# burchim/AVEC

Hardware: AMD Instinct MI355X
Metric: AV utterances/sec fwd+bwd (audio T=400, video 100x88x88) (higher is better)
Workload: dtype bf16

## Files before the change

avec_amd/csrc/wgrad_pairs.hip:

```cpp
#include "common.h"
#include "vec.h"
#include "avec_hip.h"

#ifndef WP_ABL
#define WP_ABL 0
#endif
typedef __attribute__((ext_vector_type(16))) float wp_f32x16;
typedef __attribute__((ext_vector_type(8))) __bf16 wp_bf16x8;
typedef short wp_v4s __attribute__((ext_vector_type(4)));

__device__ __attribute__((aligned(64))) unsigned char wp_zero16[64];

__device__ __forceinline__ void wp_glds16(const void* gsrc, unsigned lds_dst_uniform) {
  unsigned keep;
  asm volatile("s_mov_b32 %0, m0\n\ts_mov_b32 m0, %2\n\ts_nop 0\n\tglobal_load_lds_dwordx4 %1, off\n\ts_mov_b32 m0, %0" : "=&s"(keep) : "v"(gsrc), "s"(lds_dst_uniform) : "memory");
}
__device__ __forceinline__ uint2 wp_tr(const char* p) {
  typedef __attribute__((address_space(3))) wp_v4s* lp_t;
  return __builtin_bit_cast(uint2, __builtin_amdgcn_ds_read_tr16_b64_v4i16((lp_t)p));
}
struct WpFrag { uint2 lo, hi; };
__device__ __forceinline__ wp_f32x16 wp_mma(const WpFrag& a, const WpFrag& b, wp_f32x16 c) {
  chunk16 fa, fb; fa.w[0] = a.lo.x; fa.w[1] = a.lo.y; fa.w[2] = a.hi.x; fa.w[3] = a.hi.y; fb.w[0] = b.lo.x; fb.w[1] = b.lo.y; fb.w[2] = b.hi.x; fb.w[3] = b.hi.y;
  if (WP_ABL & 2) { asm volatile("" :: "v"(fa.w[0]), "v"(fa.w[1]), "v"(fa.w[2]), "v"(fa.w[3]), "v"(fb.w[0]), "v"(fb.w[1]), "v"(fb.w[2]), "v"(fb.w[3])); return c; }
  return __builtin_amdgcn_mfma_f32_32x32x16_bf16(__builtin_bit_cast(wp_bf16x8, fa), __builtin_bit_cast(wp_bf16x8, fb), c, 0, 0, 0);
}

struct WpArgs { const bf16* x; const bf16* dy; float* dw; int N, C, H, W; };

template <int H_, int W_, int KS_> struct WpGeom {
  static constexpr int H = H_, W = W_, KS = KS_;
  static constexpr int RWD = W | 1;
  static constexpr int RWX = W;
  static constexpr int ROWS = 16 * KS;
  static constexpr int DYB = ROWS * RWD * 128, XB = (ROWS + 2) * RWX * 256;
  static constexpr int DYI = (DYB + 1023) / 1024, XI = (XB + 1023) / 1024;
  static constexpr int DPL = (DYI + 7) / 8, XPL = (XI + 7) / 8;
  static constexpr int STAGE = (DYI + XI) * 1024;
  static constexpr int PAIRS = 3 * (3 * W - 2);
};

__device__ __forceinline__ void wp_glds16_s(unsigned voff, const void* sbase, unsigned lds_dst_uniform) {
  unsigned keep;
  asm volatile("s_mov_b32 %0, m0\n\ts_mov_b32 m0, %3\n\ts_nop 0\n\tglobal_load_lds_dwordx4 %1, %2\n\ts_mov_b32 m0, %0" : "=&s"(keep) : "v"(voff), "s"(sbase), "s"(lds_dst_uniform) : "memory");
}
template <int OFF> __device__ __forceinline__ uint2 wp_tr_o(unsigned addr) {
  static_assert(OFF >= 0 && OFF < 65536, "ds offset field");
  uint2 v; asm volatile("ds_read_b64_tr_b16 %0, %1 offset:%2" : "=v"(v) : "v"(addr), "n"(OFF) : "memory"); return v;
}

struct WpRegs { WpFrag A[4]; WpFrag B[3]; };

template <typename G, int I> struct WpIt {
  static constexpr int W = G::W, s = I / W, xp = I % W, g = s * W + xp;
  static constexpr int N0 = 2 + 2 * ((xp == 0 ? 1 : 0) + (xp + 1 < W ? 1 : 0));
  static __device__ __forceinline__ void issue0(WpRegs& R, const unsigned (&aA)[2], const unsigned (&aB)[3][2]) {
    if constexpr (xp == 0) { R.A[g & 3].lo = wp_tr_o<(16 * s * G::RWD) * 128>(aA[0]); R.A[g & 3].hi = wp_tr_o<(16 * s * G::RWD) * 128>(aA[1]); }
    if constexpr (xp + 1 < W) { R.A[(g + 1) & 3].lo = wp_tr_o<(16 * s * G::RWD + xp + 1) * 128>(aA[0]); R.A[(g + 1) & 3].hi = wp_tr_o<(16 * s * G::RWD + xp + 1) * 128>(aA[1]); }
    R.B[0].lo = wp_tr_o<(16 * s * G::RWX + xp) * 256>(aB[0][0]); R.B[0].hi = wp_tr_o<(16 * s * G::RWX + xp) * 256>(aB[0][1]);
  }
  template <int KH> static __device__ __forceinline__ void issueB(WpRegs& R, const unsigned (&aB)[3][2]) {
    R.B[KH].lo = wp_tr_o<(16 * s * G::RWX + xp) * 256>(aB[KH][0]); R.B[KH].hi = wp_tr_o<(16 * s * G::RWX + xp) * 256>(aB[KH][1]);
  }
  static __device__ __forceinline__ void arrived0(WpRegs& R) {
    if constexpr (xp == 0) asm volatile("" : "+v"(R.A[g & 3].lo), "+v"(R.A[g & 3].hi));
    if constexpr (xp + 1 < W) asm volatile("" : "+v"(R.A[(g + 1) & 3].lo), "+v"(R.A[(g + 1) & 3].hi));
    asm volatile("" : "+v"(R.B[0].lo), "+v"(R.B[0].hi));
  }
};

template <typename G, int I>
__device__ __forceinline__ void wp_iter(WpRegs& R, wp_f32x16 (&acc)[9], unsigned (&m0)[4], unsigned (&m2)[4], const int oyb, const bool hi_half, const unsigned (&aA)[2], const unsigned (&aB)[3][2]) {
  typedef WpIt<G, I> It;
  constexpr int H = G::H, W = G::W, NIT = G::KS * W, g = It::g;
  constexpr bool more = I + 1 < NIT;
  constexpr int N0N = more ? WpIt<G, more ? I + 1 : I>::N0 : 0;
  if constexpr (It::xp == 0) {
    constexpr unsigned PAT = 1u | (1u << H) | (2 * H < 16 ? 1u << ((2 * H) & 15) : 0u) | (3 * H < 16 ? 1u << ((3 * H) & 15) : 0u) | (4 * H < 16 ? 1u << ((4 * H) & 15) : 0u);
    unsigned ml0[2][4], ml2[2][4];
#pragma unroll
    for (int hh = 0; hh < 2; ++hh) {
      int bs = oyb + (8 * hh + 16 * It::s) % H; bs = bs >= H ? bs - H : bs;
      const int e0 = bs == 0 ? 0 : H - bs, e2 = e0 == 0 ? H - 1 : e0 - 1;
      const unsigned b0 = (WP_ABL & 8) ? 0u : (PAT << e0), b2 = (WP_ABL & 8) ? 0u : (PAT << e2);
#pragma unroll
      for (int dd = 0; dd < 4; ++dd) {
        ml0[hh][dd] = ~((((b0 >> (2 * dd)) & 1u) * 0xffffu) | (((b0 >> (2 * dd + 1)) & 1u) * 0xffff0000u));
        ml2[hh][dd] = ~((((b2 >> (2 * dd)) & 1u) * 0xffffu) | (((b2 >> (2 * dd + 1)) & 1u) * 0xffff0000u));
      }
    }
#pragma unroll
    for (int dd = 0; dd < 4; ++dd) { m0[dd] = hi_half ? ml0[1][dd] : ml0[0][dd]; m2[dd] = hi_half ? ml2[1][dd] : ml2[0][dd]; }
  }
  asm volatile("s_waitcnt lgkmcnt(4)" ::: "memory");
  It::arrived0(R);
  R.B[0].lo.x &= m0[0]; R.B[0].lo.y &= m0[1]; R.B[0].hi.x &= m0[2]; R.B[0].hi.y &= m0[3];
  if constexpr (It::xp + 1 < W) acc[0] = wp_mma(R.A[(g + 1) & 3], R.B[0], acc[0]);
  acc[1] = wp_mma(R.A[g & 3], R.B[0], acc[1]);
  if constexpr (It::xp >= 1) acc[2] = wp_mma(R.A[(g - 1) & 3], R.B[0], acc[2]);
  __builtin_amdgcn_sched_barrier(0);
  if constexpr (more) WpIt<G, more ? I + 1 : I>::issue0(R, aA, aB);
  asm volatile("s_waitcnt lgkmcnt(%0)" ::"n"(2 + N0N) : "memory");
  asm volatile("" : "+v"(R.B[1].lo), "+v"(R.B[1].hi));
  if constexpr (It::xp + 1 < W) acc[3] = wp_mma(R.A[(g + 1) & 3], R.B[1], acc[3]);
  acc[4] = wp_mma(R.A[g & 3], R.B[1], acc[4]);
  if constexpr (It::xp >= 1) acc[5] = wp_mma(R.A[(g - 1) & 3], R.B[1], acc[5]);
  __builtin_amdgcn_sched_barrier(0);
  if constexpr (more) WpIt<G, more ? I + 1 : I>::template issueB<1>(R, aB);
  asm volatile("s_waitcnt lgkmcnt(%0)" ::"n"(more ? N0N + 2 : 0) : "memory");
  asm volatile("" : "+v"(R.B[2].lo), "+v"(R.B[2].hi));
  R.B[2].lo.x &= m2[0]; R.B[2].lo.y &= m2[1]; R.B[2].hi.x &= m2[2]; R.B[2].hi.y &= m2[3];
  if constexpr (It::xp + 1 < W) acc[6] = wp_mma(R.A[(g + 1) & 3], R.B[2], acc[6]);
  acc[7] = wp_mma(R.A[g & 3], R.B[2], acc[7]);
  if constexpr (It::xp >= 1) acc[8] = wp_mma(R.A[(g - 1) & 3], R.B[2], acc[8]);
  __builtin_amdgcn_sched_barrier(0);
  if constexpr (more) { WpIt<G, more ? I + 1 : I>::template issueB<2>(R, aB); wp_iter<G, more ? I + 1 : I>(R, acc, m0, m2, oyb, hi_half, aA, aB); }
}

template <typename G>
__device__ __attribute__((noinline)) void wp_body(const WpArgs a_, char* const smem_, const int kind_, const int s_begin_, const int s_end_) {
  constexpr int H = G::H, W = G::W, RWD = G::RWD, RWX = G::RWX, ROWS = G::ROWS;
  auto uni = [](const void* p) { const unsigned long long v = (unsigned long long)p;
    return (const void*)(((unsigned long long)(unsigned)__builtin_amdgcn_readfirstlane((int)(v >> 32)) << 32) | (unsigned)__builtin_amdgcn_readfirstlane((int)(unsigned)v)); };
  WpArgs a; a.x = (const bf16*)uni(a_.x); a.dy = (const bf16*)uni(a_.dy); a.dw = (float*)uni(a_.dw);
  a.N = __builtin_amdgcn_readfirstlane(a_.N); a.C = __builtin_amdgcn_readfirstlane(a_.C); a.H = a_.H; a.W = a_.W;
  char* const smem = (char*)uni(smem_);
  const int kind = __builtin_amdgcn_readfirstlane(kind_), s_begin = __builtin_amdgcn_readfirstlane(s_begin_), s_end = __builtin_amdgcn_readfirstlane(s_end_);
  const int tid = threadIdx.x, lane = tid & 63, wave = __builtin_amdgcn_readfirstlane(tid >> 6);
  const int C = a.C;
  const int nci = C >> 7, cog = kind / nci, cig = kind - cog * nci;
  typedef __attribute__((address_space(3))) void* lptr_t;
  const unsigned lds0 = (unsigned)(uintptr_t)(lptr_t)smem;
  const int NR = a.N * H;

  unsigned dpl[G::DPL], xpl[G::XPL];
  auto dslot = [&](const int k, int& rr, bool& used) {
    const int S = (wave + 8 * k) * 64 + lane, pix = S >> 3, cpos = S & 7;
    rr = pix / RWD; const int xx = pix - rr * RWD, c = cpos ^ (4 * ((rr >> 1) & 1));
    used = rr < ROWS && xx < W;
    return (unsigned)(((rr * W + xx) * C + cog * 64 + c * 8) * 2);
  };
  auto xslot = [&](const int k, int& rr, bool& used) {
    const int S = (wave + 8 * k) * 64 + lane, pix = S >> 4, cpos = S & 15;
    rr = pix / RWX; const int xx = pix - rr * RWX, c = cpos ^ (4 * (rr & 3));
    used = rr < ROWS + 2;
    return (unsigned)(((rr * W + xx) * C + cig * 128 + c * 8) * 2);
  };
#pragma unroll
  for (int k = 0; k < G::DPL; ++k) { int rr; bool u; const unsigned o = dslot(k, rr, u); dpl[k] = u ? o : 0u; }
#pragma unroll
  for (int k = 0; k < G::XPL; ++k) { int rr; bool u; const unsigned o = xslot(k, rr, u); xpl[k] = u ? o : 0u; }
  auto load_stage = [&](const int q, const int par) {
    const int rs = q * ROWS;
    const unsigned d0 = lds0 + par * G::STAGE, x0 = d0 + G::DYI * 1024;
    const char* dyb = (const char*)(a.dy + (long long)rs * W * C); const char* xb = (const char*)(a.x + (long long)(rs - 1) * W * C);
    if (rs >= 1 && rs + ROWS + 1 <= NR) {
#pragma unroll
      for (int k = 0; k < G::DPL; ++k) { if (wave + 8 * k >= G::DYI) break; wp_glds16_s(dpl[k], dyb, d0 + (wave + 8 * k) * 1024); }
#pragma unroll
      for (int k = 0; k < G::XPL; ++k) { if (wave + 8 * k >= G::XI) break; wp_glds16_s(xpl[k], xb, x0 + (wave + 8 * k) * 1024); }
    } else {
#pragma unroll
      for (int k = 0; k < G::DPL; ++k) {
        if (wave + 8 * k >= G::DYI) break;
        int rr; bool u; const unsigned o = dslot(k, rr, u);
        wp_glds16((u && rs + rr < NR) ? (const void*)(dyb + o) : (const void*)wp_zero16, d0 + (wave + 8 * k) * 1024);
      }
#pragma unroll
      for (int k = 0; k < G::XPL; ++k) {
        if (wave + 8 * k >= G::XI) break;
        int rr; bool u; const unsigned o = xslot(k, rr, u); const int r = rs - 1 + rr;
        wp_glds16((u && r >= 0 && r < NR) ? (const void*)(xb + o) : (const void*)wp_zero16, x0 + (wave + 8 * k) * 1024);
      }
    }
  };

  const int cot = wave & 1, ciq = wave >> 1;
  const int g4 = lane >> 4, t = lane & 15;
  unsigned aA[2], aB[3][2];
#pragma unroll
  for (int h = 0; h < 2; ++h) {
    const int krow = 8 * (g4 >> 1) + 4 * h + (t >> 2);
    aA[h] = lds0 + krow * RWD * 128 + (((2 * cot + (g4 & 1)) ^ (2 * ((krow >> 1) & 1))) << 5) + (t & 3) * 8;
#pragma unroll
    for (int kh = 0; kh < 3; ++kh) {
      const int rr = krow + kh;
      aB[kh][h] = lds0 + G::DYI * 1024 + rr * RWX * 256 + (((2 * ciq + (g4 & 1)) ^ (2 * (rr & 3))) << 5) + (t & 3) * 8;
    }
  }
  wp_f32x16 acc[9];
#pragma unroll
  for (int j = 0; j < 9; ++j)
#pragma unroll
    for (int r = 0; r < 16; ++r) acc[j][r] = 0.f;

  int q = s_begin;
  int par = 0;
  load_stage(q, 0);
  for (; q < s_end; ++q, par ^= 1) {
    asm volatile("s_waitcnt vmcnt(0)" ::: "memory");
    __builtin_amdgcn_s_barrier();
    asm volatile("" ::: "memory");
    WpRegs R; unsigned m0[4], m2[4];
    WpIt<G, 0>::issue0(R, aA, aB); WpIt<G, 0>::template issueB<1>(R, aB); WpIt<G, 0>::template issueB<2>(R, aB);
    if (q + 1 < s_end && !(WP_ABL & 1)) load_stage(q + 1, par ^ 1);
    const int oyb = (int)(((unsigned)q * (unsigned)ROWS) % (unsigned)H);
    wp_iter<G, 0>(R, acc, m0, m2, oyb, lane >= 32, aA, aB);
    const unsigned dlt = par ? (unsigned)-G::STAGE : (unsigned)G::STAGE;
#pragma unroll
    for (int h = 0; h < 2; ++h) { aA[h] += dlt; aB[0][h] += dlt; aB[1][h] += dlt; aB[2][h] += dlt; }
  }
#pragma unroll
  for (int j = 0; j < 9; ++j)
#pragma unroll
    for (int r = 0; r < 16; ++r) {
      const int co = cog * 64 + cot * 32 + (r & 3) + 8 * (r >> 2) + 4 * (lane >> 5), ci = cig * 128 + ciq * 32 + (lane & 31);
      if (WP_ABL & 4) { if (acc[j][r] == 1234.5f) a.dw[(long long)co * 9 * C + j * C + ci] = acc[j][r]; } else
      atomicAdd(a.dw + (long long)co * 9 * C + j * C + ci, acc[j][r]);
    }
  __builtin_amdgcn_s_barrier();
}

typedef WpGeom<11, 11, 1> WpG11;
typedef WpGeom<6, 6, 2> WpG6;
typedef WpGeom<3, 3, 4> WpG3;
static constexpr size_t wp_max3(size_t a, size_t b, size_t c) { return a > b ? (a > c ? a : c) : (b > c ? b : c); }
static constexpr size_t WP_LDS = wp_max3(2 * WpG11::STAGE, 2 * WpG6::STAGE, 2 * WpG3::STAGE);
static_assert(WP_LDS <= 160 * 1024, "two stages must fit the LDS");

struct WpGroup { WpArgs it[AVEC_WGRAD_GROUP_MAX]; long long cum[AVEC_WGRAD_GROUP_MAX + 1]; int stages[AVEC_WGRAD_GROUP_MAX], wt[AVEC_WGRAD_GROUP_MAX], ranges[AVEC_WGRAD_GROUP_MAX]; int n; };
__global__ __launch_bounds__(512) void wgrad3x3_pairs_grouped_kernel(WpGroup grp) {
  extern __shared__ __attribute__((aligned(16))) char smem[];
  const long long T = grp.cum[grp.n];
  const int nb = (int)gridDim.x, per = nb >> 3;
  const int slot = (nb & 7) ? (int)blockIdx.x : ((int)blockIdx.x & 7) * per + ((int)blockIdx.x >> 3);
  const long long lo = T * (long long)slot / nb, hi = T * (long long)(slot + 1) / nb;
  for (int i = 0; i < grp.n; ++i) {
    const long long c0 = grp.cum[i], c1 = grp.cum[i + 1];
    if (hi <= c0 || lo >= c1) continue;
    const WpArgs& a = grp.it[i];
    const int nst = grp.stages[i], wt = grp.wt[i], R = grp.ranges[i], kinds = (a.C >> 6) * (a.C >> 7);
    long long u = ((lo > c0 ? lo : c0) - c0) / wt; const long long u1 = ((hi < c1 ? hi : c1) - c0) / wt;
    while (u < u1) {
      int r = (int)((u / kinds) * R / nst); if (r >= R) r = R - 1;
      while (r + 1 < R && (long long)kinds * (int)((long long)(r + 1) * nst / R) <= u) ++r;
      while (r > 0 && (long long)kinds * (int)((long long)r * nst / R) > u) --r;
      const int rs0 = (int)((long long)r * nst / R), rs1 = (int)((long long)(r + 1) * nst / R), len = rs1 - rs0;
      const long long v = u - (long long)kinds * rs0;
      const int k = (int)(v / len), sb = rs0 + (int)(v % len);
      long long take = rs1 - sb; if (take > u1 - u) take = u1 - u;
      const int se = sb + (int)take;
      if (a.W == 11) wp_body<WpG11>(a, smem, k, sb, se);
      else if (a.W == 6) wp_body<WpG6>(a, smem, k, sb, se);
      else wp_body<WpG3>(a, smem, k, sb, se);
      u += take;
    }
  }
}

bool wgrad3x3_pairs_supported(int H, int W, int C) {
  static const bool off = getenv("AVEC_NO_WGRAD_PAIRS") != nullptr;
  return !off && C >= 128 && C % 128 == 0 && C <= 1024 && ((H == 11 && W == 11) || (H == 6 && W == 6) || (H == 3 && W == 3));
}

template <typename G> static constexpr int wp_stage_weight() {
  return (G::KS * (G::PAIRS * 64 + 8 * G::W * 32) + 512) / 64;
}
int wgrad3x3_pairs_grouped(const avec_wgrad3x3_item_t* items, int n, hipStream_t st) {
  WpGroup g; g.n = n; g.cum[0] = 0;
  long long total_stages = 0;
  for (int i = 0; i < n; ++i) {
    const avec_wgrad3x3_item_t& t = items[i];
    WpArgs& a = g.it[i]; a.x = (const bf16*)t.x; a.dy = (const bf16*)t.dy; a.dw = t.dw; a.N = (int)t.images; a.C = t.C; a.H = t.H; a.W = t.W;
    AVEC_CHECK_ARG(t.images * t.H < (1ll << 26) && 70ll * t.W * t.C * 2 < (1ll << 31), "wgrad3x3_pairs: item %d too large", i);
    const int rows = t.W == 11 ? WpG11::ROWS : t.W == 6 ? WpG6::ROWS : WpG3::ROWS;
    g.wt[i] = t.W == 11 ? wp_stage_weight<WpG11>() : t.W == 6 ? wp_stage_weight<WpG6>() : wp_stage_weight<WpG3>();
    g.stages[i] = (int)((t.images * t.H + rows - 1) / rows);
    const int kinds = (t.C / 64) * (t.C / 128);
    g.cum[i + 1] = g.cum[i] + (long long)kinds * g.stages[i] * g.wt[i];
    total_stages += (long long)kinds * g.stages[i];
  }
  const int grid = (int)(total_stages < 256 ? total_stages : 256);
  for (int i = 0; i < n; ++i) {
    const int kinds = (items[i].C / 64) * (items[i].C / 128);
    const double shares = (double)grid * (double)(g.cum[i + 1] - g.cum[i]) / (double)g.cum[n];
    int R = (int)(shares / kinds + 0.5); if (R < 1) R = 1; if (R > g.stages[i]) R = g.stages[i];
    g.ranges[i] = R;
  }
  if (int r = avec_lds_optin(wgrad3x3_pairs_grouped_kernel, WP_LDS)) return r;
  avec_note_kernel("wgrad3x3_pairs_grouped_kernel");
  hipLaunchKernelGGL(wgrad3x3_pairs_grouped_kernel, dim3((unsigned)grid), dim3(512), WP_LDS, st, g);
  AVEC_LAUNCH_CHECK();
  return 0;
}

#ifdef WP_PROBE
extern __shared__ __attribute__((aligned(16))) char wp_probe_smem[];
__global__ __launch_bounds__(512) void wp_probe11(WpArgs a) { wp_body<WpG11>(a, wp_probe_smem, blockIdx.x, 0, gridDim.x); }
__global__ __launch_bounds__(512) void wp_probe6(WpArgs a) { wp_body<WpG6>(a, wp_probe_smem, blockIdx.x, 0, gridDim.x); }
__global__ __launch_bounds__(512) void wp_probe3(WpArgs a) { wp_body<WpG3>(a, wp_probe_smem, blockIdx.x, 0, gridDim.x); }
#endif
```

Baseline: 1832.

## Schedule grouped wgrad work as XCD-local teams sharing stage ranges

```diff
diff --git a/avec_amd/csrc/wgrad_pairs.hip b/avec_amd/csrc/wgrad_pairs.hip
--- a/avec_amd/csrc/wgrad_pairs.hip
+++ b/avec_amd/csrc/wgrad_pairs.hip
@@ -1,6 +1,9 @@
 #include "common.h"
 #include "vec.h"
 #include "avec_hip.h"
+#define WP_PLAN_FN __host__ __device__ inline
+#define WP_PLAN_MAX_ITEMS AVEC_WGRAD_GROUP_MAX
+#include "wgrad_pairs_plan.h"
 
 #ifndef WP_ABL
 #define WP_ABL 0
@@ -227,10 +230,25 @@
 static constexpr size_t wp_max3(size_t a, size_t b, size_t c) { return a > b ? (a > c ? a : c) : (b > c ? b : c); }
 static constexpr size_t WP_LDS = wp_max3(2 * WpG11::STAGE, 2 * WpG6::STAGE, 2 * WpG3::STAGE);
 static_assert(WP_LDS <= 160 * 1024, "two stages must fit the LDS");
-
-struct WpGroup { WpArgs it[AVEC_WGRAD_GROUP_MAX]; long long cum[AVEC_WGRAD_GROUP_MAX + 1]; int stages[AVEC_WGRAD_GROUP_MAX], wt[AVEC_WGRAD_GROUP_MAX], ranges[AVEC_WGRAD_GROUP_MAX]; int n; };
+static_assert(wp_stage_rows(11) == WpG11::ROWS && wp_stage_rows(6) == WpG6::ROWS && wp_stage_rows(3) == WpG3::ROWS, "wgrad_pairs_plan.h counts stages of these geometries");
+
+__device__ __forceinline__ void wp_run(const WpArgs& a, char* const smem, const int kind, const int s_begin, const int s_end) {
+  if (a.W == 11) wp_body<WpG11>(a, smem, kind, s_begin, s_end);
+  else if (a.W == 6) wp_body<WpG6>(a, smem, kind, s_begin, s_end);
+  else wp_body<WpG3>(a, smem, kind, s_begin, s_end);
+}
+
+struct WpGroup {
+  WpArgs it[AVEC_WGRAD_GROUP_MAX]; long long cum[AVEC_WGRAD_GROUP_MAX + 1]; int stages[AVEC_WGRAD_GROUP_MAX], wt[AVEC_WGRAD_GROUP_MAX], ranges[AVEC_WGRAD_GROUP_MAX], kinds[AVEC_WGRAD_GROUP_MAX];
+  WpTeamPlan team; int teams; int n;
+};
+static_assert(sizeof(WpGroup) < 4096, "kernel argument block");
 __global__ __launch_bounds__(512) void wgrad3x3_pairs_grouped_kernel(WpGroup grp) {
   extern __shared__ __attribute__((aligned(16))) char smem[];
+  if (grp.teams) {
+    wp_team_segments(grp.team, grp.kinds, grp.stages, grp.n, (int)blockIdx.x, [&](const int i, const int k, const int sb, const int se) { wp_run(grp.it[i], smem, k, sb, se); });
+    return;
+  }
   const long long T = grp.cum[grp.n];
   const int nb = (int)gridDim.x, per = nb >> 3;
   const int slot = (nb & 7) ? (int)blockIdx.x : ((int)blockIdx.x & 7) * per + ((int)blockIdx.x >> 3);
@@ -250,9 +268,7 @@
       const int k = (int)(v / len), sb = rs0 + (int)(v % len);
       long long take = rs1 - sb; if (take > u1 - u) take = u1 - u;
       const int se = sb + (int)take;
-      if (a.W == 11) wp_body<WpG11>(a, smem, k, sb, se);
-      else if (a.W == 6) wp_body<WpG6>(a, smem, k, sb, se);
-      else wp_body<WpG3>(a, smem, k, sb, se);
+      wp_run(a, smem, k, sb, se);
       u += take;
     }
   }
@@ -263,24 +279,23 @@
   return !off && C >= 128 && C % 128 == 0 && C <= 1024 && ((H == 11 && W == 11) || (H == 6 && W == 6) || (H == 3 && W == 3));
 }
 
-template <typename G> static constexpr int wp_stage_weight() {
-  return (G::KS * (G::PAIRS * 64 + 8 * G::W * 32) + 512) / 64;
-}
+template <typename G> static constexpr int wp_weight_of() { return (G::KS * (G::PAIRS * 64 + 8 * G::W * 32) + 512) / 64; }
+static_assert(wp_stage_weight(11) == wp_weight_of<WpG11>() && wp_stage_weight(6) == wp_weight_of<WpG6>() && wp_stage_weight(3) == wp_weight_of<WpG3>(), "wgrad_pairs_plan.h restates the cost of a stage");
 int wgrad3x3_pairs_grouped(const avec_wgrad3x3_item_t* items, int n, hipStream_t st) {
   WpGroup g; g.n = n; g.cum[0] = 0;
-  long long total_stages = 0;
   for (int i = 0; i < n; ++i) {
     const avec_wgrad3x3_item_t& t = items[i];
     WpArgs& a = g.it[i]; a.x = (const bf16*)t.x; a.dy = (const bf16*)t.dy; a.dw = t.dw; a.N = (int)t.images; a.C = t.C; a.H = t.H; a.W = t.W;
     AVEC_CHECK_ARG(t.images * t.H < (1ll << 26) && 70ll * t.W * t.C * 2 < (1ll << 31), "wgrad3x3_pairs: item %d too large", i);
-    const int rows = t.W == 11 ? WpG11::ROWS : t.W == 6 ? WpG6::ROWS : WpG3::ROWS;
-    g.wt[i] = t.W == 11 ? wp_stage_weight<WpG11>() : t.W == 6 ? wp_stage_weight<WpG6>() : wp_stage_weight<WpG3>();
-    g.stages[i] = (int)((t.images * t.H + rows - 1) / rows);
-    const int kinds = (t.C / 64) * (t.C / 128);
+    g.wt[i] = wp_stage_weight(t.W);
+    g.stages[i] = wp_stages(t.images, t.H, t.W);
+    const int kinds = g.kinds[i] = wp_kinds(t.C);
     g.cum[i + 1] = g.cum[i] + (long long)kinds * g.stages[i] * g.wt[i];
-    total_stages += (long long)kinds * g.stages[i];
-  }
-  const int grid = (int)(total_stages < 256 ? total_stages : 256);
+  }
+  const int grid = wp_grid(g.kinds, g.stages, n);
+  int width[AVEC_WGRAD_GROUP_MAX];
+  for (int i = 0; i < n; ++i) width[i] = items[i].W;
+  g.teams = getenv("AVEC_NO_WGRAD_TEAMS") == nullptr && wp_team_plan(g.kinds, g.stages, width, n, grid, g.team);
   for (int i = 0; i < n; ++i) {
     const int kinds = (items[i].C / 64) * (items[i].C / 128);
     const double shares = (double)grid * (double)(g.cum[i + 1] - g.cum[i]) / (double)g.cum[n];
diff --git a/avec_amd/csrc/wgrad_pairs_plan.h b/avec_amd/csrc/wgrad_pairs_plan.h
--- /dev/null
+++ b/avec_amd/csrc/wgrad_pairs_plan.h
@@ -0,0 +1,68 @@
+#pragma once
+
+#ifndef WP_PLAN_FN
+#define WP_PLAN_FN inline
+#endif
+#ifndef WP_PLAN_MAX_ITEMS
+#define WP_PLAN_MAX_ITEMS 16
+#endif
+
+constexpr int WP_TEAM_GRID = 256;
+constexpr int WP_TEAM_PHASES = 3;
+
+struct WpTeamPlan { int xs[WP_TEAM_PHASES][9]; };
+
+WP_PLAN_FN constexpr int wp_stage_rows(const int W) { return W == 11 ? 16 : W == 6 ? 32 : 64; }
+WP_PLAN_FN constexpr int wp_stage_weight(const int W) { return ((wp_stage_rows(W) / 16) * (3 * (3 * W - 2) * 64 + 8 * W * 32) + 512) / 64; }
+WP_PLAN_FN int wp_stages(const long long images, const int H, const int W) { return (int)((images * H + wp_stage_rows(W) - 1) / wp_stage_rows(W)); }
+WP_PLAN_FN int wp_grid(const int* kinds, const int* stages, const int n) {
+  long long units = 0;
+  for (int i = 0; i < n; ++i) units += (long long)kinds[i] * stages[i];
+  return (int)(units < WP_TEAM_GRID ? units : WP_TEAM_GRID);
+}
+WP_PLAN_FN int wp_kinds(const int C) { return (C >> 6) * (C >> 7); }
+WP_PLAN_FN int wp_team_phase(const int kinds) { return kinds == 32 ? 0 : kinds == 8 ? 1 : kinds == 2 ? 2 : -1; }
+
+WP_PLAN_FN bool wp_team_plan(const int* kinds, const int* stages, const int* width, const int n, const int grid, WpTeamPlan& plan) {
+  int w[WP_TEAM_PHASES] = {0, 0, 0};
+  long long tot[WP_TEAM_PHASES] = {0, 0, 0}, unit[WP_TEAM_PHASES], start[WP_TEAM_PHASES], C = 0;
+  for (int p = 0; p < WP_TEAM_PHASES; ++p)
+    for (int x = 0; x <= 8; ++x) plan.xs[p][x] = 0;
+  if (grid != WP_TEAM_GRID || n < 1 || n > WP_PLAN_MAX_ITEMS) return false;
+  for (int i = 0; i < n; ++i) {
+    const int p = wp_team_phase(kinds[i]);
+    if (p < 0 || stages[i] < 1) return false;
+    if (w[p] && w[p] != width[i]) return false;
+    w[p] = width[i]; tot[p] += stages[i];
+  }
+  for (int p = 0; p < WP_TEAM_PHASES; ++p) {
+    if (tot[p] >= (1ll << 30)) return false;
+    unit[p] = tot[p] ? (long long)(32 >> (2 * p)) * wp_stage_weight(w[p]) : 1;
+    start[p] = C; C += unit[p] * tot[p];
+  }
+  for (int x = 0; x <= 8; ++x)
+    for (int p = 0; p < WP_TEAM_PHASES; ++p) {
+      const long long rel = C * x / 8 - start[p];
+      long long s = rel <= 0 ? 0 : (rel + unit[p] / 2) / unit[p];
+      plan.xs[p][x] = (int)(s > tot[p] ? tot[p] : s);
+    }
+  return true;
+}
+
+template <typename F>
+WP_PLAN_FN void wp_team_segments(const WpTeamPlan& plan, const int* kinds, const int* stages, const int n, const int wg, F&& f) {
+  const int xcd = wg & 7, j = wg >> 3;
+  for (int p = 0; p < WP_TEAM_PHASES; ++p) {
+    const int first = plan.xs[p][xcd], count = plan.xs[p][xcd + 1] - first;
+    if (count <= 0) continue;
+    const int K = 32 >> (2 * p), teams = 32 / K, team = j / K, member = j - team * K;
+    const int lo = first + (int)((long long)count * team / teams), hi = first + (int)((long long)count * (team + 1) / teams);
+    int off = 0;
+    for (int i = 0; i < n && off < hi; ++i) {
+      if (kinds[i] != K) continue;
+      const int b = (lo > off ? lo : off) - off, e = (hi < off + stages[i] ? hi : off + stages[i]) - off;
+      if (b < e) f(i, member, b, e);
+      off += stages[i];
+    }
+  }
+}
```

Measured after the change: 1836, median of 6. Within noise of the previous version (+0.2%).
